# KenHBS/LDA_thesis

Measured on AMD Instinct MI355X. Metric: million tokens resampled/sec (Gibbs sweep), higher is better.
Workload: dtype f64-exact (fp32 tier 0 + fp64 tiers: the drawn topic is the fp64 pipeline's)

## Files before the change

### lda_thesis_amd/csrc/kernel_quad.hpp

```cpp
#pragma once

namespace {

constexpr float LLDA_MARGIN0_QUAD = 0x1.ap-18f;
constexpr float QM_L = 1.05f * 32.0f * 0x1p-24f, QM_T = 1.05f * 39.0f * 0x1p-24f, QM_P = 1.05f * 37.0f * 0x1p-24f, QM_TOT = 1.05f * 0.25f * 0x1p-24f;
#define QLDS(arr, rho, t) (arr)[(rho) >> 2][t][(rho) & 3]
constexpr int QT = 32;
#ifdef LLDA_QUAD_PRIO
constexpr int QP_TOP = (LLDA_QUAD_PRIO) / 100 % 10, QP_DEC = (LLDA_QUAD_PRIO) / 10 % 10, QP_BULK = (LLDA_QUAD_PRIO) % 10;
#else
constexpr int QP_TOP = 3, QP_DEC = 0, QP_BULK = 2;
#endif
constexpr int QNT = 128;
#ifdef LLDA_QUAD_PARTS
constexpr int QUAD_PARTS = (LLDA_QUAD_PARTS);
#else
constexpr int QUAD_PARTS = 7;
#endif
constexpr bool QUAD_FULL_LOOP = (QUAD_PARTS & 1) != 0, QUAD_HOOKS_OUT = (QUAD_PARTS & 2) != 0, QUAD_EARLY_DECODE = (QUAD_PARTS & 4) != 0;
template <bool B> struct QuadForm { static constexpr bool value = B; };

template <int LB>
struct QuadGeo {
    static constexpr int LPD = 1 << LB;
    static constexpr int G = 2 * LPD;
    static constexpr int KP = 32 * LPD;
    static constexpr int IS = 3 + LB;
    static constexpr int DPW = 64 / LPD;
    static constexpr uint64_t GM = LPD == 64 ? ~0ull : ((1ull << LPD) - 1);
    static constexpr uint32_t KEY_NONE = 0xFC000u | 31u << 9 | (uint32_t)(KP - 1);
};

template <int LB>
__device__ __forceinline__ int quad_rho(int pos) { return ((pos >> LB) & 0x18) | ((pos & 3) << 1) | ((pos >> 2) & 1); }
constexpr int quad_rho_of(int i, int e, int c) { return 8 * i + 2 * c + e; }

template <int LB>
__device__ __forceinline__ uint32_t quad_min_key(uint32_t key)
{
    if constexpr (LB == 4)
        asm volatile("s_nop 1\n\tv_min_u32_dpp %0, %0, %0 row_ror:8 row_mask:0xf bank_mask:0xf\n\ts_nop 1\n\t"
                     "v_min_u32_dpp %0, %0, %0 row_ror:4 row_mask:0xf bank_mask:0xf\n\ts_nop 1\n\t"
                     "v_min_u32_dpp %0, %0, %0 row_ror:2 row_mask:0xf bank_mask:0xf\n\ts_nop 1\n\t"
                     "v_min_u32_dpp %0, %0, %0 row_ror:1 row_mask:0xf bank_mask:0xf" : "+v"(key));
    else if constexpr (LB == 3)
        asm volatile("s_nop 1\n\tv_min_u32_dpp %0, %0, %0 row_half_mirror row_mask:0xf bank_mask:0xf\n\ts_nop 1\n\t"
                     "v_min_u32_dpp %0, %0, %0 quad_perm:[1,0,3,2] row_mask:0xf bank_mask:0xf\n\ts_nop 1\n\t"
                     "v_min_u32_dpp %0, %0, %0 quad_perm:[2,3,0,1] row_mask:0xf bank_mask:0xf" : "+v"(key));
    else
        asm volatile("s_nop 1\n\tv_min_u32_dpp %0, %0, %0 quad_perm:[1,0,3,2] row_mask:0xf bank_mask:0xf\n\ts_nop 1\n\t"
                     "v_min_u32_dpp %0, %0, %0 quad_perm:[2,3,0,1] row_mask:0xf bank_mask:0xf" : "+v"(key));
    return key;
}

template <int LB>
struct QuadCounts {
    const int (*s_ndk)[QNT][4];
    const int *s_nk0;
    int t;
    int e;
    int g;
    bool st;
    __device__ __forceinline__ int word(int s) const { return QLDS(s_ndk, 8 * (s >> 2) + 2 * (s & 3) + e, t); }
    __device__ __forceinline__ int nd(int s) const { return word(s) & 0xffff; }
    __device__ __forceinline__ int nk(int s) const
    {
        const int w = word(s);
        return s_nk0[pos_of<QuadGeo<LB>::G, 16>(g, s)] + (w & 0xffff) - (int)((uint32_t)w >> 16);
    }
    __device__ __forceinline__ bool stats() const { return st; }
    __device__ __forceinline__ bool count_unsure() const { return false; }
};

template <int LB, bool PAD>
__device__ __noinline__ int quad_cold(const int (*s_ndk)[QNT][4], const int *s_nk0, int tbase, int w, int f, int zo, uint32_t ra,
                                      uint32_t rb, int lane, int64_t d, const KParams *P)
{
    constexpr int G = QuadGeo<LB>::G;
    const int g = lane & (G - 1);
    int x[16];
    gload_lane_row<G, 16>(P->n_kw, (int64_t)w * QuadGeo<LB>::KP, g, x);
    int lo, so;
    lane_slot_of<G, 16>(zo, lo, so);
#pragma unroll
    for (int s = 0; s < 16; ++s) x[s] -= (g == lo && s == so) ? f : 0;
    const QuadCounts<LB> dc{s_ndk, s_nk0, tbase + (g >> 1), g & 1, g, lane < G};
    if constexpr (PAD) return cold_tiers_acc<G, 16, true, false>(dc, x, P->lab_mask[d * G + g], uniform53(ra, rb), g, lane, P);
    else return cold_tiers_acc<G, 16, false, true>(dc, x, 0xFFFFu, uniform53(ra, rb), g, lane, P);
// ... 29 lines not shown
        tot += dpp_f32<DPP_ROW_ROR + 8>(tot);
        tot += dpp_f32<DPP_ROW_ROR + 4>(tot);
        tot += dpp_f32<DPP_ROW_ROR + 2>(tot);
        tot += dpp_f32<DPP_ROW_ROR + 1>(tot);
        prev = __int_as_float(__builtin_amdgcn_update_dpp(0, __float_as_int(X), DPP_ROW_SHR + 1, 0xF, 0xF, true));
    } else {
        const float m1 = lq >= 1 ? 1.0f : 0.0f, m2 = lq >= 2 ? 1.0f : 0.0f;
        X = __builtin_fmaf(dpp_f32<DPP_ROW_SHR + 1>(X), m1, X);
        X = __builtin_fmaf(dpp_f32<DPP_ROW_SHR + 2>(X), m2, X);
        if constexpr (LB == 3) {
            const float m4 = lq >= 4 ? 1.0f : 0.0f;
            X = __builtin_fmaf(dpp_f32<DPP_ROW_SHR + 4>(X), m4, X);
            tot += dpp_f32<DPP_HALF_MIRROR>(tot);
        }
        tot += dpp_f32<DPP_XOR1>(tot);
        tot += dpp_f32<DPP_XOR2>(tot);
        prev = dpp_f32<DPP_ROW_SHR + 1>(X) * m1;
    }
    LLDA_MARK("threshold");
    const float t = u * tot;
    const float tg = t - prev;
    const float md = __builtin_fmaf(QM_L, X0, __builtin_fmaf(QM_T, t, __builtin_fmaf(QM_P, prev, QM_TOT * tot)));
    float margin = md;
    if constexpr (HOOKS) margin = __builtin_fmaf(tot, margin_rel, margin_data * md);
    const float lo0 = tg - margin, hi0 = tg + margin;
    LLDA_MARK("search");
    const bool c0 = Q[15].x <= lo0;
    const float dA = c0 ? Q[15].x : 0.0f;
    const float lo = lo0 - dA, hi = hi0 - dA;
    float q[16];
#pragma unroll
    for (int a = 0; a < 16; ++a) q[a] = c0 ? Q[a].y : Q[a].x;
    const bool c5 = q[15] <= lo;
    float ub = c5 ? __int_as_float(0x7f800000) : q[15];
    const bool c1 = q[7] <= lo;
    ub = c1 ? ub : q[7];
    const float m2 = c1 ? q[11] : q[3];
    const float a1 = c1 ? q[9] : q[1], a5 = c1 ? q[13] : q[5];
    const float e0 = c1 ? q[8] : q[0], e2 = c1 ? q[10] : q[2], e4 = c1 ? q[12] : q[4], e6 = c1 ? q[14] : q[6];
    const bool c2 = m2 <= lo;
    ub = c2 ? ub : m2;
    const float m3 = c2 ? a5 : a1;
    const float g0 = c2 ? e4 : e0, g2 = c2 ? e6 : e2;
    const bool c3 = m3 <= lo;
    ub = c3 ? ub : m3;
    const float m4 = c3 ? g2 : g0;
    const bool c4 = m4 <= lo;
    ub = c4 ? ub : m4;
    uint64_t bad_total;
    asm("v_cmp_class_f32_e64 %0, %1, %2" : "=s"(bad_total) : "v"(tot - margin), "v"(0x2FF));
    uint64_t unsure = __ballot(!(ub > hi)) | bad_total;
    LLDA_MARK("pick");
    constexpr uint32_t I1 = 2u << QuadGeo<LB>::IS, I0 = 1u << QuadGeo<LB>::IS;
    const uint32_t p = (c1 ? (I1 | 16u << 9) : 0u) | (c2 ? (I0 | 8u << 9) : 0u) | (c3 ? (2u | 4u << 9) : 0u) | (c4 ? (1u | 2u << 9) : 0u) |
                       (c0 ? (4u | 1u << 9) : 0u) | ((uint32_t)lq << 3) | ((uint32_t)lq << 14);
    uint32_t key = c5 ? QuadGeo<LB>::KEY_NONE : p;
    key = quad_min_key<LB>(key);
    zn = (int)(key & 0x3FFFu);
    if constexpr (PAD) unsure |= __ballot(key == QuadGeo<LB>::KEY_NONE);
    return unsure;
}

template <int LB, bool PAD = false>
__device__ __forceinline__ uint64_t quad_tier1(const q_v32f &xv, const int (*s_ndk)[QNT][4], const int *s_nk0, int tid, int lq, double u,
                                               double alpha, double beta, double vbeta, double margin_rel, uint32_t vm, int &zn)
{
    double W[QT];
    double run = 0.0;
#pragma unroll
    for (int k = 0; k < QT; ++k) {
        const int e = k >> 4, a = k & 15, i = a >> 2, c = a & 3;
        const int rho = quad_rho_of(i, e, c);
        const int w = QLDS(s_ndk, rho, tid);
        const int nd = w & 0xffff, nk = s_nk0[(i << QuadGeo<LB>::IS) | (lq << 3) | (e << 2) | c] + nd - (int)((uint32_t)w >> 16);
        const double den = (double)nk + vbeta;
        double y = (double)__builtin_amdgcn_rcpf((float)den);
        y = __builtin_fma(__builtin_fma(-den, y, 1.0), y, y);
        y = __builtin_fma(__builtin_fma(-den, y, 1.0), y, y);
        const double ws = ((double)nd + alpha) * (((double)xv[rho] + beta) * y);
        run = run + (((vm >> k) & 1u) ? ws : 0.0);
        W[k] = run;
    }
    constexpr int LPD = QuadGeo<LB>::LPD;
    const double X = group_scan<LPD>(run, lq);
    const double tot = bcast_last<LPD>(X, tid & 63);
    double prev = dpp_f64<DPP_ROW_SHR + 1>(X);
    if constexpr (LB < 4) prev = lq ? prev : 0.0;
    const double tg = u * tot - prev;
    const double margin = tot * margin_rel;
    const double lo = tg - margin, hi = tg + margin;
    int cnt_lo = 0, cnt_hi = 0;
#pragma unroll
    for (int k = 0; k < QT; ++k) {
        cnt_lo += (W[k] <= lo) ? 1 : 0;
        cnt_hi += (W[k] <= hi) ? 1 : 0;
    }
    uint64_t unsure = __ballot((cnt_lo != cnt_hi) || !(tot > 0.0) || !(margin < tot));
    const uint32_t k = (uint32_t)cnt_lo;
    const uint32_t i_ = (k >> 2) & 3u, e_ = (k >> 4) & 1u, c_ = k & 3u;
    const uint32_t p = (i_ << QuadGeo<LB>::IS) | ((uint32_t)lq << 3) | (e_ << 2) | c_ | ((8u * i_ + 2u * c_ + e_) << 9) | ((uint32_t)lq << 14);
    uint32_t key = cnt_lo >= QT ? QuadGeo<LB>::KEY_NONE : p;
    key = quad_min_key<LB>(key);
    zn = (int)(key & 0x3FFFu);
    if constexpr (PAD) unsure |= __ballot(key == QuadGeo<LB>::KEY_NONE);
    return unsure;
}

struct QuadSite { int v, f, zo, c, zn, lo, so; uint8_t w; };

#ifdef QUAD_PROFILE
#define QP_DECL uint32_t qp_t = 0, qp_acc[8] = {0, 0, 0, 0, 0, 0, 0, 0}
#define QP_START() do { __builtin_amdgcn_sched_barrier(0); qp_t = (uint32_t)__builtin_amdgcn_s_memtime(); __builtin_amdgcn_sched_barrier(0); } while (0)
#define QP_MARK(k) do { __builtin_amdgcn_sched_barrier(0); const uint32_t qp_n = (uint32_t)__builtin_amdgcn_s_memtime(); \
                        qp_acc[k] += qp_n - qp_t; qp_t = qp_n; __builtin_amdgcn_sched_barrier(0); } while (0)
#else
#define QP_DECL
#define QP_START()
#define QP_MARK(k)
#endif

template <int LB, bool REC = (LB < 4), bool PAD = false, bool HOOKS = false>
__global__ void __launch_bounds__(QNT, 2) llda_sweep_quad_kernel(const KParams P)
{
    typedef QuadGeo<LB> Geo;
    constexpr int KP = Geo::KP, LPD = Geo::LPD, G = Geo::G, IS = Geo::IS;
    __shared__ int s_nk[KP];
    __shared__ int s_nk0[KP];
    __shared__ int s_ndk[QT / 4][QNT][4];
    __shared__ float s_pa[QT / 4][QNT][4];
    __shared__ float s_u[QNT / LPD][2 * LPD];
    __shared__ __attribute__((aligned(16))) int s_hot[QT][16];
    static_assert(LB != 4 || sizeof(s_nk) + sizeof(s_nk0) + sizeof(s_ndk) + sizeof(s_pa) + sizeof(s_u) + sizeof(s_hot) <= 40960,
                  "K = 512: the static LDS of a workgroup must leave room for four workgroups on a CU");

    const int tid = threadIdx.x;
    for (int i = tid; i < KP; i += QNT) {
        s_nk[i] = 0;
        s_nk0[i] = P.n_k[i];
    }
    for (int i = tid; i < QT * 16; i += QNT) {
        const int so = i >> 4, k = i & 15;
        const int kk = ((so & 1) << 3) | ((so >> 4) << 2) | (((so >> 3) & 1) << 1) | ((so >> 2) & 1);
        s_hot[so][k] = k == kk ? -(1 << (((so >> 1) & 1) << 4)) : 0;
    }
    __syncthreads();

    const int lane = tid & 63, lq = tid & (LPD - 1), row = lane >> LB, grp = tid >> LB;
    const int gbase = lane & (64 - LPD);
    const float vbeta32 = (float)P.vbeta, alpha32 = (float)P.alpha, beta32 = (float)P.beta;

    const int64_t site_base = P.doc_off[0];
    const int32_t *word_b = P.word + site_base, *freq_b = P.freq + site_base, *csc_b = P.csc_pos + site_base;
    int32_t *z_b = P.z + site_base;

    typedef int v4i __attribute__((ext_vector_type(4)));
    QP_DECL;

    auto update = [&](int sg, int pos, int df) {
        const int w = QLDS(s_ndk, sg, tid) + df;
        QLDS(s_ndk, sg, tid) = w;
        const int nd = w & 0xffff, nk = s_nk0[pos] + nd - (int)((uint32_t)w >> 16);
        QLDS(s_pa, sg, tid) = tier0_factor(nd, nk, alpha32, vbeta32);
    };

    for (int it = 0; it < P.dpg; ++it) {
        const int64_t idx = ((int64_t)blockIdx.x * P.dpg + it) * (QNT / LPD) + grp;
        const bool valid = idx < P.D;
        const int64_t ic = valid ? idx : P.D - 1;
        const int64_t d = P.doc_order ? (int64_t)P.doc_order[ic] : ic;
        int64_t s0 = P.doc_off[d];
        int len = valid ? (int)(P.doc_off[d + 1] - s0) : 0;
        if (len <= 0) {
            len = 0;
            s0 = site_base;
        }
        int maxlen, minlen;
        if constexpr (LB == 4) {
            const int l0 = __builtin_amdgcn_readlane(len, 0), l1 = __builtin_amdgcn_readlane(len, 16);
            const int l2 = __builtin_amdgcn_readlane(len, 32), l3 = __builtin_amdgcn_readlane(len, 48);
            maxlen = max(max(l0, l1), max(l2, l3));
            minlen = min(min(l0, l1), min(l2, l3));
        } else {
            int ml = len, nl = len;
#pragma unroll
            for (int m = LPD; m < 64; m <<= 1) {
                ml = max(ml, __shfl_xor(ml, m, 64));
                nl = min(nl, __shfl_xor(nl, m, 64));
            }
            maxlen = __builtin_amdgcn_readfirstlane(ml);
            minlen = __builtin_amdgcn_readfirstlane(nl);
        }
        if (maxlen == 0) continue;

        int32_t *ndk_row = P.n_dk + d * KP;
        const uint32_t vm = PAD ? (uint32_t)P.lab_mask[d * G + 2 * lq] | (uint32_t)P.lab_mask[d * G + 2 * lq + 1] << 16 : ~0u;
        {
            int big = 0, tokens = 0;
#pragma unroll
            for (int i = 0; i < 4; ++i) {
                const v4i a = ((const v4i *)ndk_row)[i * G + 2 * lq], b = ((const v4i *)ndk_row)[i * G + 2 * lq + 1];
                const int r[8] = {a.x, a.y, a.z, a.w, b.x, b.y, b.z, b.w};
#pragma unroll
                for (int j = 0; j < 8; ++j) {
                    const int rho = quad_rho_of(i, j >> 2, j & 3);
                    const int k = s_nk0[(i << IS) + lq * 8 + j];
                    QLDS(s_ndk, rho, tid) = r[j] | (r[j] << 16);
                    QLDS(s_pa, rho, tid) = ((vm >> (16 * (j >> 2) + 4 * i + (j & 3))) & 1u) ? tier0_factor(r[j], k, alpha32, vbeta32) : 0.0f;
                    big |= r[j];
                    tokens += (int)((uint32_t)r[j] & 0xffffu);
                }
            }
#pragma unroll
            for (int m = 1; m < LPD; m <<= 1) tokens += __shfl_xor(tokens, m, LPD);
            if (valid && (((uint32_t)big >> 16) || tokens > 65535) && P.status) atomicOr(P.status, 4);
        }
        const uint32_t gdoc = (uint32_t)(d + P.doc_base);
        const uint32_t sb = (uint32_t)(s0 - site_base) * 4u;
        const int last = len > 0 ? len - 1 : 0;
        auto off_of = [&](int n) { return opaque_u32(sb + (uint32_t)min(n, last) * 4u); };
        auto off_full = [&](int n) { return opaque_u32(sb + (uint32_t)n * 4u); };
        auto load_scalars = [&](QuadSite &R, const uint32_t o) {
            R.v = gload_i32(word_b, o); R.f = gload_i32(freq_b, o); R.c = gload_i32(csc_b, o); R.zo = gload_i32(z_b, o);
        };
        const int32_t *rec_b = REC ? P.site_rec + site_base * 4 : nullptr;
        int pv = 0, pf = 0, pc = 0;
        auto load_rec = [&](int &v, int &f, int &c, const uint32_t o) {
            const v4i r = *(const LLDA_GLOBAL v4i *)((const LLDA_GLOBAL char *)rec_b + (o << 2));
            v = r.x; f = r.y; c = r.z;
        };
        auto decode_old = [&](QuadSite &R) {
            R.lo = (R.zo >> 3) & (LPD - 1);
            R.so = quad_rho<LB>(R.zo);
        };
        int xp[16];
        auto load_row16 = [&](const int v, uint8_t &flag) {
#ifdef ABL_NOLOAD
#pragma unroll
            for (int k = 0; k < 16; ++k) xp[k] = ((v + k) & 7) * 0x10001;
            flag = 1;
            return;
#endif
            const LLDA_GLOBAL char *q = (const LLDA_GLOBAL char *)P.n_kw16 + (((uint32_t)v << (IS + 3)) + (uint32_t)lq * 16u);
            const v4i a = *(const LLDA_GLOBAL v4i *)q, b = *(const LLDA_GLOBAL v4i *)(q + 32 * LPD);
            const v4i c = *(const LLDA_GLOBAL v4i *)(q + 16 * LPD), e = *(const LLDA_GLOBAL v4i *)(q + 48 * LPD);
            xp[0] = a.x; xp[1] = a.y; xp[2] = a.z; xp[3] = a.w;
            xp[4] = b.x; xp[5] = b.y; xp[6] = b.z; xp[7] = b.w;
            xp[8] = c.x; xp[9] = c.y; xp[10] = c.z; xp[11] = c.w;
            xp[12] = e.x; xp[13] = e.y; xp[14] = e.z; xp[15] = e.w;
            flag = *(const LLDA_GLOBAL uint8_t *)((const LLDA_GLOBAL char *)P.row16 + (uint32_t)v);
        };
        q_v32f xv;
        auto convert_row = [&](const int v, const uint8_t flag, const int so, const float own) {
            LLDA_MARK("convert");
            const uint64_t wide_w = __ballot(flag == 0);
            if (__builtin_expect(wide_w == 0, 1)) {
#pragma unroll
                for (int k = 0; k < 16; ++k) {
                    const int e = k >> 3, j = (k >> 2) & 1, m = k & 3;
                    const int i = 2 * j + (m >> 1), c = 2 * (m & 1);
                    xv[quad_rho_of(i, e, c)] = (float)((uint32_t)xp[k] & 0xffffu);
                    xv[quad_rho_of(i, e, c + 1)] = (float)((uint32_t)xp[k] >> 16);
                }
            } else {
                LLDA_MARK("rare_wide_row");
                int xi[QT];
#pragma unroll
                for (int t = 0; t < QT; ++t) xi[t] = 0;
                if (flag == 0) {
                    const LLDA_GLOBAL v4i *q = (const LLDA_GLOBAL v4i *)((const LLDA_GLOBAL int32_t *)P.n_kw + ((uint64_t)(uint32_t)v << (IS + 2)));
#pragma unroll
                    for (int i = 0; i < 4; ++i) {
                        const v4i a = q[i * G + 2 * lq], b = q[i * G + 2 * lq + 1];
                        xi[quad_rho_of(i, 0, 0)] = a.x; xi[quad_rho_of(i, 0, 1)] = a.y; xi[quad_rho_of(i, 0, 2)] = a.z; xi[quad_rho_of(i, 0, 3)] = a.w;
                        xi[quad_rho_of(i, 1, 0)] = b.x; xi[quad_rho_of(i, 1, 1)] = b.y; xi[quad_rho_of(i, 1, 2)] = b.z; xi[quad_rho_of(i, 1, 3)] = b.w;
                    }
                }
#pragma unroll
                for (int k = 0; k < 16; ++k) {
                    const int e = k >> 3, j = (k >> 2) & 1, m = k & 3;
                    const int i = 2 * j + (m >> 1), c = 2 * (m & 1);
                    const int ra_ = quad_rho_of(i, e, c), rb_ = quad_rho_of(i, e, c + 1);
                    xv[ra_] = flag == 0 ? (float)xi[ra_] : (float)((uint32_t)xp[k] & 0xffffu);
                    xv[rb_] = flag == 0 ? (float)xi[rb_] : (float)((uint32_t)xp[k] >> 16);
                }
#pragma unroll
                for (int r = 0; r < QT; ++r) xv[r] -= (flag == 0 && so == r) ? own : 0.0f;
            }
        };
        auto remove_own_packed = [&](const int so, const int own) {
            LLDA_MARK("own_removal");
            const v4i *hot = (const v4i *)&s_hot[so][0];
#pragma unroll
            for (int j = 0; j < 4; ++j) {
                const v4i h = hot[j];
                xp[4 * j] += __mul24(h.x, own); xp[4 * j + 1] += __mul24(h.y, own);
                xp[4 * j + 2] += __mul24(h.z, own); xp[4 * j + 3] += __mul24(h.w, own);
            }
        };

        QuadSite R0, R1, R2;
        int wq = 0;
        if constexpr (REC) {
            load_rec(R0.v, R0.f, R0.c, off_of(0)); R0.zo = gload_i32(z_b, off_of(0));
            load_rec(R1.v, R1.f, R1.c, off_of(1)); R1.zo = gload_i32(z_b, off_of(1));
            load_rec(pv, pf, pc, off_of(2));
        } else {
            load_scalars(R0, off_of(0));
            load_scalars(R1, off_of(1));
            wq = gload_i32(word_b, off_of(2));
        }
        R0.zn = R1.zn = 0;
        R2.v = R2.f = R2.zo = R2.c = R2.zn = R2.lo = R2.so = R2.w = 0;
        if constexpr (QUAD_EARLY_DECODE) {
            R2.v = REC ? pv : wq;
            R2.zo = gload_i32(z_b, off_of(2));
        }
        load_row16(R0.v, R0.w);
        uint32_t r0 = 0, r1 = 0, r2 = 0, r3 = 0;
        decode_old(R0);
        if constexpr (QUAD_EARLY_DECODE) decode_old(R1);
        if (len > 0 && lq == R0.lo) update(R0.so, R0.zo, -R0.f);
        remove_own_packed(R0.so, (len > 0 && lq == R0.lo) ? R0.f : 0);
        convert_row(R0.v, R0.w, R0.so, (len > 0 && lq == R0.lo) ? (float)R0.f : 0.0f);
        load_row16(R1.v, R1.w);

        auto site = [&](auto form, const int n, QuadSite &cur, QuadSite &nxt, QuadSite &prv) {
            constexpr bool FULL = decltype(form)::value;
            const bool act = FULL || n < len, more = FULL || n + 1 < len;
            auto off = [&](int m) { if constexpr (FULL) return off_full(m); else return off_of(m); };
            const int f = cur.f, zo = cur.zo;
            QP_START();
            if constexpr (FULL || !QUAD_FULL_LOOP) {
                LLDA_MARK("site_top");
            } else {
                LLDA_MARK("site_top_masked");
            }
            LLDA_MARK("lds_factors");
            __builtin_amdgcn_s_setprio(QP_TOP);
            q_v2f pa[16];
#pragma unroll
            for (int a = 0; a < 16; ++a) {
                pa[a].x = QLDS(s_pa, 2 * a, tid);
                pa[a].y = QLDS(s_pa, 2 * a + 1, tid);
            }
            LLDA_MARK("rng");
            if ((n & (2 * LPD - 1)) == 0) {
                LLDA_MARK("rare_philox");
                r0 = (uint32_t)(n >> 1) + (uint32_t)lq; r1 = gdoc; r2 = P.stream_id; r3 = P.sweep;
                philox4x32_10(r0, r1, r2, r3, P.key0, P.key1);
                s_u[grp][2 * lq] = (float)(r0 >> 5) * 0x1p-27f;
                s_u[grp][2 * lq + 1] = (float)(r2 >> 5) * 0x1p-27f;
                LLDA_MARK("rng");
            }
            const float u32 = s_u[grp][n & (2 * LPD - 1)];
            QP_MARK(0);
            int zn;
            uint64_t unsure;
            if constexpr (HOOKS) unsure = quad_draw<LB, PAD, true>(xv, pa, u32, P.margin0_rel, P.margin0_data, beta32, lq, zn);
            else unsure = quad_draw<LB, PAD, false>(xv, pa, u32, 0.0f, 1.0f, beta32, lq, zn);
            if constexpr (!FULL) unsure &= __ballot(act);
            QP_MARK(1);
            LLDA_MARK("cold_check");
            if (__builtin_expect(unsure != 0, 0)) {
                LLDA_MARK("rare_cold");
                const int holder = (n >> 1) & (LPD - 1);
                const uint32_t ra_l = (n & 1) ? r2 : r0, rb_l = (n & 1) ? r3 : r1;
                const int bp_h = (gbase | holder) << 2;
                const uint32_t ra = (uint32_t)__builtin_amdgcn_ds_bpermute(bp_h, (int)ra_l), rb = (uint32_t)__builtin_amdgcn_ds_bpermute(bp_h, (int)rb_l);
                const uint64_t t0_w = unsure;
                if (lq == 0 && ((t0_w >> gbase) & Geo::GM) && P.status) atomicAdd(P.status + 1, 1);
                int z1;
                uint64_t still = ((!HOOKS || P.margin_rel < 1.0 ? quad_tier1<LB, PAD>(xv, s_ndk, s_nk0, tid, lq, uniform53(ra, rb), P.alpha, P.beta, P.vbeta,
                                                                                  P.margin_rel, vm, z1) : ~0ull) | __ballot(cur.w == 0));
                if constexpr (!FULL) still &= __ballot(act);
                const bool mine0 = ((t0_w >> gbase) & Geo::GM) != 0;
                zn = mine0 ? z1 : zn;
                uint32_t rows = 0;
#pragma unroll
                for (int r = 0; r < Geo::DPW; ++r)
                    rows |= (((t0_w >> (LPD * r)) & Geo::GM) && ((still >> (LPD * r)) & Geo::GM)) ? (1u << r) : 0u;
                rows = (uint32_t)__builtin_amdgcn_readfirstlane((int)rows);
                while (__builtin_expect(rows != 0, 0)) {
                    const int r = __builtin_ctz(rows);
                    rows &= rows - 1;
                    const int src = r * LPD;
                    const int zo_r = __builtin_amdgcn_readlane(zo, src);
                    int zc = quad_cold<LB, PAD>(s_ndk, s_nk0, (tid & 64) + src, __builtin_amdgcn_readlane(cur.v, src),
                                       __builtin_amdgcn_readlane(f, src), zo_r, (uint32_t)__builtin_amdgcn_readlane((int)ra, src),
                                       (uint32_t)__builtin_amdgcn_readlane((int)rb, src), lane,
                                       (int64_t)__builtin_amdgcn_readlane((int)d, src),
                                       (const KParams *)__builtin_amdgcn_kernarg_segment_ptr());
                    if (__builtin_expect(zc < 0, 0)) {
                        zc = zo_r;
                        if (lane == 0 && P.status) atomicOr(P.status, 1);
                    }
                    zn = (row == r) ? (zc | (quad_rho<LB>(zc) << 9)) : zn;
                }
            }
            QP_MARK(2);
            LLDA_MARK("decode");

            {
                const int zpos = zn & 511, sn = zn >> 9, ln = (zn >> 3) & (LPD - 1);
                cur.zn = zpos;
                uint32_t cword = (uint32_t)zo | ((uint32_t)zpos << 16);
                asm volatile("" : "+v"(cword));
                if constexpr (!QUAD_EARLY_DECODE) decode_old(nxt);
                const bool own_new = act && lq == ln, own_old = more && lq == nxt.lo;
                const int sg = own_new ? sn : own_old ? nxt.so : 0;
                const int ps = own_new ? zpos : own_old ? nxt.zo : (lq << 3);
                const int df = own_new ? f : own_old ? -nxt.f : 0;
                LLDA_MARK("count_update");
                const int w0 = QLDS(s_ndk, sg, tid), k0 = s_nk0[ps];
                QP_MARK(3);
                LLDA_MARK("scalars");
                __builtin_amdgcn_s_setprio(QP_BULK);
                int w_next;
                if constexpr (REC) {
                    prv.v = w_next = pv; prv.f = pf; prv.c = pc;
                    if constexpr (QUAD_EARLY_DECODE) cur.zo = gload_i32(z_b, off(n + 3));
                    else prv.zo = gload_i32(z_b, off(n + 2));
                    load_rec(pv, pf, pc, off(n + 3));
                } else if constexpr (QUAD_EARLY_DECODE) {
                    w_next = prv.v;
                    prv.f = gload_i32(freq_b, off(n + 2)); prv.c = gload_i32(csc_b, off(n + 2));
                    cur.v = gload_i32(word_b, off(n + 3)); cur.zo = gload_i32(z_b, off(n + 3));
                } else {
                    w_next = wq;
                    load_scalars(prv, off(n + 2));
                    wq = gload_i32(word_b, off(n + 3));
                }
                if constexpr (QUAD_EARLY_DECODE) decode_old(prv);
                QP_MARK(4);
                remove_own_packed(nxt.so, (more && lq == nxt.lo) ? nxt.f : 0);
                convert_row(nxt.v, nxt.w, nxt.so, (more && lq == nxt.lo) ? (float)nxt.f : 0.0f);
                QP_MARK(5);
                LLDA_MARK("row_prefetch");
                load_row16(w_next, prv.w);
                LLDA_MARK("count_update");
                const int w = w0 + df;
                QLDS(s_ndk, sg, tid) = w;
                const int nd = w & 0xffff, nk = k0 + nd - (int)((uint32_t)w >> 16);
                QLDS(s_pa, sg, tid) = tier0_factor(nd, nk, alpha32, vbeta32);
                if (__builtin_expect(__ballot(own_new && own_old) != 0, 0)) {
                    LLDA_MARK("rare_second_update");
                    if (own_new && own_old) update(nxt.so, nxt.zo, -nxt.f);
                }
#ifndef ABL_NOCOMMIT
                {
                    LLDA_MARK("commit");
                    const uint32_t zoff = opaque_u32(sb + (uint32_t)n * 4u);
                    const LLDA_GLOBAL uint32_t *lp = (const LLDA_GLOBAL uint32_t *)P.commit_log + (uint32_t)(cur.c & 0x7fffffff);
                    const uint32_t word = cword;
                    if (lq == 0 && act) {
                        gstore_i32(z_b, zoff, zpos);
                        *(LLDA_GLOBAL uint32_t *)lp = word;
                    }
                }
#endif
            }
            LLDA_MARK("loop");
            QP_MARK(6);
        };
        int n = 0;
        if constexpr (QUAD_FULL_LOOP) {
            for (; n + 5 < minlen; n += 3) {
                site(QuadForm<true>{}, n, R0, R1, R2);
                site(QuadForm<true>{}, n + 1, R1, R2, R0);
                site(QuadForm<true>{}, n + 2, R2, R0, R1);
            }
        }
        for (;; n += 3) {
            site(QuadForm<false>{}, n, R0, R1, R2);
            if (n + 1 >= maxlen) break;
            site(QuadForm<false>{}, n + 1, R1, R2, R0);
            if (n + 2 >= maxlen) break;
            site(QuadForm<false>{}, n + 2, R2, R0, R1);
            if (n + 3 >= maxlen) break;
        }

#ifdef QUAD_PROFILE
        if (blockIdx.x == 0 && tid == 0 && P.status) {
#pragma unroll
            for (int k = 0; k < 8; ++k) atomicAdd(P.status + 8 + k, (int)qp_acc[k]);
            atomicAdd(P.status + 16, maxlen);
        }
#endif
        if (valid && len > 0) {
#pragma unroll
            for (int i = 0; i < 4; ++i) {
                int o[8];
#pragma unroll
                for (int j = 0; j < 8; ++j) {
                    const int w = QLDS(s_ndk, quad_rho_of(i, j >> 2, j & 3), tid);
                    o[j] = w & 0xffff;
                    const int dl = o[j] - (int)((uint32_t)w >> 16);
                    if (dl) atomicAdd(&s_nk[(i << IS) + lq * 8 + j], dl);
                }
                v4i a = {o[0], o[1], o[2], o[3]}, b = {o[4], o[5], o[6], o[7]};
                ((v4i *)ndk_row)[i * G + 2 * lq] = a;
                ((v4i *)ndk_row)[i * G + 2 * lq + 1] = b;
            }
        }
    }

    __syncthreads();
    for (int i = tid; i < KP; i += QNT) {
        const int dl = s_nk[i];
        if (dl) atomicAdd(P.n_k_delta + i, dl);
// ... 28 lines not shown
```

### lda_thesis_amd/csrc/llda_gibbs.hip

```cpp
#include <hip/hip_runtime.h>
#include "build_info.hpp"
#ifndef ABL_EXTRA_LDS_BYTES
#define ABL_EXTRA_LDS_BYTES 0
#endif
#include <stdint.h>
#include <math.h>
#include <string.h>
#include <map>
#include <memory>
#include <type_traits>

#include "llda_gibbs.h"

#pragma clang fp contract(off)

#include "device_common.hpp"
#include "draw_tiers.hpp"
#include "exact_generic.hpp"
#include "kernel_sweep.hpp"
#include "kernel_quad.hpp"
#include "kernel_sparse.hpp"
#include "kernel_batch.hpp"
#include "kernel_readout.hpp"
#include "kernel_foldin.hpp"
// ... 503 lines not shown
            rl = allow_lds(llda_sweep_wide_kernel<true>, lds);
            if (rl) return rl;
            hipLaunchKernelGGL(llda_sweep_wide_kernel<true>, grid, block, lds, st, W);
        } else {
            rl = allow_lds(llda_sweep_wide_kernel<false>, lds);
            if (rl) return rl;
            hipLaunchKernelGGL(llda_sweep_wide_kernel<false>, grid, block, lds, st, W);
        }
#undef LLDA_WIDE_REG
        const hipError_t e = hipGetLastError();
        return e == hipSuccess ? LLDA_OK : hip_fail(e);
    }

    const bool sparse = fast && !dense && a->live_off && a->live_pos && a->live_max >= 1 && a->live_max <= LLDA_MAX_LIVE;
    const int G = sparse ? (a->live_max <= 8 ? 8 : a->live_max <= 16 ? 16 : a->live_max <= 32 ? 32 : 64) : L.G;
    const int gpb = 256 / G;
    int dpg = a->docs_per_group;
    if (dpg < 1) dpg = 1;
    P.dpg = dpg;
    const int64_t per_block = (int64_t)gpb * dpg;
    const int64_t blocks = (a->D + per_block - 1) / per_block;
    if (blocks > 0x7fffffffLL) return LLDA_E_BAD_ARG;

    if (sparse) {
        P.live_off = a->live_off; P.live_pos = a->live_pos;
        if (a->debug_margin < 0) {
            P.margin_rel = 2.0;
            P.margin0_rel = 2.0f;
        }
        const dim3 grid((unsigned)blocks), block(256);
        const int rimg = take_image(a, P);
        if (rimg) return rimg;
#define LLDA_SPARSE(GS_)                                                                                              \
    case GS_:                                                                                                         \
        if (a->img_bits == 8) hipLaunchKernelGGL((llda_sweep_sparse_kernel<GS_, KParams, 8>), grid, block, 0, st, P);       \
        else if (a->img_bits == 16) hipLaunchKernelGGL((llda_sweep_sparse_kernel<GS_, KParams, 16>), grid, block, 0, st, P); \
        else hipLaunchKernelGGL((llda_sweep_sparse_kernel<GS_, KParams, 0>), grid, block, 0, st, P);                       \
        break;
        switch (G) { LLDA_SPARSE(8) LLDA_SPARSE(16) LLDA_SPARSE(32) LLDA_SPARSE(64) }
#undef LLDA_SPARSE
        const hipError_t e = hipGetLastError();
        return e == hipSuccess ? LLDA_OK : hip_fail(e);
    }
    if (a->n_kw_img || a->img_bits) return LLDA_E_BAD_ARG;
    if (a->row16) {
        if (!a->n_kw16 || a->site_row) return LLDA_E_BAD_ARG;
        if (!(fast && a->dense_mask != 0 && logged && llda_quad_ok(a->K))) return LLDA_E_BAD_ARG;
        if (a->D >= (1LL << 31)) return LLDA_E_BAD_ARG;
        P.quad_pad = L.K != L.KP;
        if (P.quad_pad && !P.lab_mask) return LLDA_E_BAD_ARG;
        if (!(a->max_doc_tokens > 0 && a->max_doc_tokens < 65536)) return LLDA_E_BAD_ARG;
        if ((reinterpret_cast<uintptr_t>(a->n_kw16) | reinterpret_cast<uintptr_t>(a->n_kw)) & 15) return LLDA_E_BAD_ARG;
        if (a->V >= (1LL << 22)) return LLDA_E_BAD_ARG;
        if (L.G <= 16 && !P.site_rec) return LLDA_E_BAD_ARG;
        if (a->n_sites < 1) return LLDA_OK;
        P.n_kw16 = a->n_kw16;
        P.row16 = a->row16;
        if (a->debug_margin == 0) {
            P.margin0_rel = 0.0f;
            P.margin0_data = 1.0f;
        } else if (a->debug_margin == -9) {
            P.margin0_rel = LLDA_MARGIN0_QUAD;
            P.margin_rel = 0x1p-40;
        } else if (a->debug_margin <= -10 && a->debug_margin >= -18) {
            P.margin0_rel = 0.0f;
            P.margin0_data = a->debug_margin == -10 ? 1.0f / 1.05f : ldexpf(1.0f, a->debug_margin + 10);
            P.margin_rel = 0x1p-40;
        }
        const int64_t per_q = (int64_t)(2 * QNT / L.G) * dpg;
        const int64_t qblocks = (a->D + per_q - 1) / per_q;
        if (qblocks > 0x7fffffffLL) return LLDA_E_BAD_ARG;
        const dim3 qgrid((unsigned)qblocks), qblock(QNT);
        const bool hooks = a->debug_margin != 0 || !QUAD_HOOKS_OUT;
#define LLDA_QUAD(LB_, REC_, PAD_)                                                                                                    \
        do {                                                                                                                           \
            if (hooks) hipLaunchKernelGGL((llda_sweep_quad_kernel<LB_, REC_, PAD_, true>), qgrid, qblock, 0, st, P);                   \
            else hipLaunchKernelGGL((llda_sweep_quad_kernel<LB_, REC_, PAD_, false>), qgrid, qblock, 0, st, P);                        \
        } while (0)
        if (!P.quad_pad) {
            if (L.G == 32) LLDA_QUAD(4, false, false);
            else if (L.G == 16) LLDA_QUAD(3, true, false);
            else LLDA_QUAD(2, true, false);
        } else {
            if (L.G == 32) LLDA_QUAD(4, false, true);
            else if (L.G == 16) LLDA_QUAD(3, true, true);
            else LLDA_QUAD(2, true, true);
        }
#undef LLDA_QUAD
        const hipError_t e = hipGetLastError();
        return e == hipSuccess ? LLDA_OK : hip_fail(e);
    }
    if ((a->n_kw16 != nullptr) != (a->site_row != nullptr)) return LLDA_E_BAD_ARG;
    if (a->n_kw16) {
        if (!(fast && dense && logged && L.T == 16 && L.G >= 32)) return LLDA_E_BAD_ARG;
        if ((reinterpret_cast<uintptr_t>(a->n_kw16) | reinterpret_cast<uintptr_t>(a->n_kw)) & 15) return LLDA_E_BAD_ARG;
        P.n_kw16 = a->n_kw16;
        P.site_row = a->site_row;
        P.w4 = a->max_doc_tokens > 0 && a->max_doc_tokens < 65536 && a->debug_margin != -8;
    }
    switch (L.G) {
    case 8: return dispatch_sweep_T<8>(L.T, P, has_tail, fast, dense, blocks, st);
    case 16: return dispatch_sweep_T<16>(L.T, P, has_tail, fast, dense, blocks, st);
    case 32: return dispatch_sweep_T<32>(L.T, P, has_tail, fast, dense, blocks, st);
    case 64: return dispatch_sweep_T<64>(L.T, P, has_tail, fast, dense, blocks, st);
    }
    return LLDA_E_BAD_K;
// ... 367 lines not shown
```

### lda_thesis_amd/sampler.py

```python
import os

import numpy as np
import torch

from . import _native
from .layout import group_layout


def shard_documents(doc_off, world_size):
    doc_off = np.asarray(doc_off, dtype=np.int64)
    D = doc_off.shape[0] - 1
    total = int(doc_off[-1])
    bounds = [0]
    for r in range(1, world_size):
        target = total * r // world_size
        b = int(np.searchsorted(doc_off, target, side="left"))
        bounds.append(min(max(b, bounds[-1]), D))
    bounds.append(D)
    return bounds


def _dist_active(group):
    import torch.distributed as dist
    return dist.is_available() and dist.is_initialized() and dist.get_world_size(group) > 1
# ... 218 lines not shown
        def lines_per_site(column):
            n_lines = (KP + per_line - 1) // per_line
            key = torch.unique(docs * n_lines + column // per_line)
            per_doc = torch.bincount(key // n_lines, minlength=self.D).to(torch.float32)
            return float((per_doc * lens).sum().item() / max(float(lens.sum().item()), 1.0))
        self.image_lines_per_site = (lines_per_site(pos), lines_per_site(col_t[pos]))
        if force is not True and self.image_lines_per_site[1] > 0.9 * self.image_lines_per_site[0]:
            return
        self._img_src = torch.from_numpy(src.astype(np.int32)).to(dev)
        self._img_col = col_t.to(torch.int32)

    QUAD_MAX_WIDE_SITES = 0.02
    QUAD_CHECK_EVERY = 32

    def _quad_policy(self):
        if self.sweeps_done % self.QUAD_CHECK_EVERY:
            return
        ev = self._wide_event
        if ev is not None:
            ev.synchronize()
            self._wide_event = None
            if float(self._wide_host[0]) > self.QUAD_MAX_WIDE_SITES * self.S:
                self.quad = False
                self.row16 = None
                if _native.rows16_ok(self.K):
                    self._flag_rows16()
                else:
                    self.n_kw16 = None
                return
        if self._wide_host is None:
            self._wide_host = torch.zeros((1,), dtype=torch.float32).pin_memory()
        share = ((1.0 - self.row16.to(torch.float32)) * self._word_sites).sum().reshape(1)
        self._wide_host.copy_(share, non_blocking=True)
        self._wide_event = torch.cuda.Event()
        self._wide_event.record()

    ROWS16_MIN_BYTES = 64 << 20
    MAX_FREQ = 1 << 23
    PAIR_LIMIT = 32767

    def _make_rows16(self, auto=False):
        V, KP = self.V, self.layout.KP
        if KP % 8:
            raise _native.NativeError("llda_rows16_ok(%d) holds but KP = %d is not a multiple of 8" % (self.K, KP))
        if (V + 1) * (KP // 4) + V * (KP // 8) >= 1 << 31:
            if auto:
                return
            raise ValueError("rows16=True: n_kw of %d x %d is too large for the 32-bit row offsets of the 16-bit-row kernel"
                             % (V, KP))
        tokens_max = int(min(int(self.n_dk.sum(dim=1, dtype=torch.int64).max().item()), 2 ** 31 - 1)) if self.D else 0
        four_waves = 0 < tokens_max < 65536
        if auto and not four_waves and V * KP * 4 < self.ROWS16_MIN_BYTES:
            return
        quad = bool(self._quad_wanted is not False and four_waves and _native.quad_ok(self.K) and V < (1 << 22))
        two_doc = _native.rows16_ok(self.K)
        if quad and self._quad_wanted is None:
            wide = (self.n_kw.max(dim=1).values > 65535) | (self.n_kw.min(dim=1).values < 0)
            self._word_sites = torch.bincount(self.word.to(torch.int64), minlength=V).to(torch.float32)
            if float((wide.to(torch.float32) * self._word_sites).sum().item()) > self.QUAD_MAX_WIDE_SITES * self.S:
                quad = False
        if self._quad_wanted and not quad:
            raise ValueError("quad=True: needs a K with llda_quad_ok (16 slots per lane in 8, 16 or 32 lanes: K = 100, 128, 200, 256, 400, 512 ...), "
                             "documents of fewer than 65 536 tokens and a vocabulary below 2^22 words")
        if not quad and not (two_doc and bool(self._rows16_fits().any())):
            return
        n32 = (V + 1) * KP
        try:
            both = torch.zeros((n32 + V * KP // 2,), dtype=torch.int32, device=self.device)
        except torch.cuda.OutOfMemoryError:
            if not auto:
                raise
            import warnings
            warnings.warn("GibbsSampler: no room for the 16-bit image of n_kw (%.1f GB); sweeping with int32 rows"
                          % (V * KP * 2 / 1e9))
            return
        both[:n32] = self._counts
        self._counts = both[:n32]
        self.n_kw = self._counts[:V * KP].view(V, KP)
        self.n_k = self._counts[V * KP:]
        self._counts16 = both
        self.n_kw16 = both[n32:].view(torch.int16)
        self.quad = quad
        if self.quad:
            self.row16 = torch.zeros((V,), dtype=torch.uint8, device=self.device)
            self.max_doc_tokens = tokens_max
            return
        self._flag_rows16()
        if not self.max_doc_tokens:
            self.max_doc_tokens = tokens_max

    def _rows16_fits(self):
        return (self.n_kw.sum(dim=1, dtype=torch.int64) <= 65535) & (self.n_kw.min(dim=1).values >= 0)

    def _flag_rows16(self):
        KP = self.layout.KP
        fits = self._rows16_fits()
        self.row16 = fits.to(torch.uint8).contiguous()
        w = self.word.to(torch.int64)
        flagged = fits[w]
        self.csc_pos &= 0x7fffffff
        self.csc_pos |= torch.where(flagged, -(1 << 31), 0).to(torch.int32)
        gap = self.n_kw16.data_ptr() - self.n_kw.data_ptr()
        if gap != (self.V + 1) * KP * 4 or gap % 16:
            raise _native.NativeError("n_kw16 is not in the allocation of n_kw")
        self.site_row = torch.where(flagged, gap // 16 + w * (KP // 8), w * (KP // 4)).to(torch.int32).contiguous()

    def _make_exchange_rows(self):
        import torch.distributed as dist
        dev, KP = self.device, self.layout.KP
        mass = torch.zeros((self.V,), dtype=torch.int64, device=dev)
        if self.S:
            mass.index_add_(0, self.word.to(torch.int64), self.freq.to(torch.int64))
        everyone = torch.tensor([1 if (self.commit_log is not None or self.S == 0) else 0], device=dev)
        if _dist_active(self.group):
            dist.all_reduce(mass, group=self.group)
            dist.all_reduce(everyone, op=dist.ReduceOp.MIN, group=self.group)
# ... 412 lines not shown
```

Before: 9128.

## Encode LDS byte offsets in slot keys and use table-driven decode in quad sweep

Replaces the slot index carried in the pick key with a precomputed entry that holds the byte offsets of the count/factor pair and the hot row in LDS, so address arithmetic in the hot update and own-removal paths collapses to a mask and add. Adds an optional LDS lookup table for decoding old topics, and a small-index mode that hoists the collision ballot and uses a 32-bit commit-log offset, with a new site-count limit guarding it. It costs an extra LDS table and a wider key, and restricts quad use to fewer than 2^30 sites.

```diff
diff --git a/lda_thesis_amd/csrc/kernel_quad.hpp b/lda_thesis_amd/csrc/kernel_quad.hpp
--- a/lda_thesis_amd/csrc/kernel_quad.hpp
+++ b/lda_thesis_amd/csrc/kernel_quad.hpp
@@ -15,9 +15,10 @@
 #ifdef LLDA_QUAD_PARTS
 constexpr int QUAD_PARTS = (LLDA_QUAD_PARTS);
 #else
-constexpr int QUAD_PARTS = 7;
+constexpr int QUAD_PARTS = 55;
 #endif
 constexpr bool QUAD_FULL_LOOP = (QUAD_PARTS & 1) != 0, QUAD_HOOKS_OUT = (QUAD_PARTS & 2) != 0, QUAD_EARLY_DECODE = (QUAD_PARTS & 4) != 0;
+constexpr bool QUAD_ENTRY = (QUAD_PARTS & 8) != 0, QUAD_TABLE = (QUAD_PARTS & 16) != 0, QUAD_SMALL = (QUAD_PARTS & 32) != 0;
 template <bool B> struct QuadForm { static constexpr bool value = B; };
 
 template <int LB>
@@ -28,12 +29,35 @@
     static constexpr int IS = 3 + LB;
     static constexpr int DPW = 64 / LPD;
     static constexpr uint64_t GM = LPD == 64 ? ~0ull : ((1ull << LPD) - 1);
-    static constexpr uint32_t KEY_NONE = 0xFC000u | 31u << 9 | (uint32_t)(KP - 1);
 };
 
 template <int LB>
 __device__ __forceinline__ int quad_rho(int pos) { return ((pos >> LB) & 0x18) | ((pos & 3) << 1) | ((pos >> 2) & 1); }
 constexpr int quad_rho_of(int i, int e, int c) { return 8 * i + 2 * c + e; }
+
+constexpr uint32_t QE_NDK = 0x380Cu, QE_HOT = 0x7C0u;
+constexpr uint32_t quad_entry(uint32_t rho) { return ((rho >> 2) * 2048u + (rho & 3u) * 4u) | rho << 6; }
+constexpr uint32_t quad_slot(uint32_t rho) { return QUAD_ENTRY ? quad_entry(rho) : rho; }
+constexpr int QS_BITS = QUAD_ENTRY ? 14 : 5;
+constexpr int QK_LANE = 9 + QS_BITS;
+constexpr uint32_t QK_ZN = (1u << QK_LANE) - 1;
+template <int LB> constexpr uint32_t QUAD_KEY_NONE = 0x3Fu << QK_LANE | quad_slot(31) << 9 | (uint32_t)(QuadGeo<LB>::KP - 1);
+constexpr bool quad_entry_ok()
+{
+    uint32_t seen_or = 0;
+    for (uint32_t r = 0; r < 32; ++r) {
+        const uint32_t en = quad_entry(r);
+        if ((en & ~(QE_NDK | QE_HOT)) || (en & QE_HOT) != r << 6 || (en & QE_NDK) != (r >> 2) * 2048u + (r & 3u) * 4u) return false;
+        for (uint32_t q = 0; q < r; ++q)
+            if (quad_entry(q) == en) return false;
+        if (quad_entry(r | 1u) != (en | quad_entry(1)) || quad_entry(r | 8u) != (en | quad_entry(8))) return false;
+        seen_or |= en;
+    }
+    return seen_or == (QE_NDK | QE_HOT);
+}
+static_assert((QE_NDK & QE_HOT) == 0, "the two fields of an entry do not overlap");
+static_assert(quad_entry_ok(), "quad_entry: injective on 0 .. 31, each field recovers its offset, OR of slots = OR of entries");
+static_assert(quad_entry(31) < (1u << 14) && (0x3Fu << QK_LANE | QK_ZN) <= 0x7FFFFFFFu, "the key fits 31 bits");
 
 template <int LB>
 __device__ __forceinline__ uint32_t quad_min_key(uint32_t key)
@@ -169,12 +193,12 @@
     uint64_t unsure = __ballot(!(ub > hi)) | bad_total;
     LLDA_MARK("pick");
     constexpr uint32_t I1 = 2u << QuadGeo<LB>::IS, I0 = 1u << QuadGeo<LB>::IS;
-    const uint32_t p = (c1 ? (I1 | 16u << 9) : 0u) | (c2 ? (I0 | 8u << 9) : 0u) | (c3 ? (2u | 4u << 9) : 0u) | (c4 ? (1u | 2u << 9) : 0u) |
-                       (c0 ? (4u | 1u << 9) : 0u) | ((uint32_t)lq << 3) | ((uint32_t)lq << 14);
-    uint32_t key = c5 ? QuadGeo<LB>::KEY_NONE : p;
+    const uint32_t p = (c1 ? (I1 | quad_slot(16) << 9) : 0u) | (c2 ? (I0 | quad_slot(8) << 9) : 0u) | (c3 ? (2u | quad_slot(4) << 9) : 0u) |
+                       (c4 ? (1u | quad_slot(2) << 9) : 0u) | (c0 ? (4u | quad_slot(1) << 9) : 0u) | ((uint32_t)lq << 3) | ((uint32_t)lq << QK_LANE);
+    uint32_t key = c5 ? QUAD_KEY_NONE<LB> : p;
     key = quad_min_key<LB>(key);
-    zn = (int)(key & 0x3FFFu);
-    if constexpr (PAD) unsure |= __ballot(key == QuadGeo<LB>::KEY_NONE);
+    zn = (int)(key & QK_ZN);
+    if constexpr (PAD) unsure |= __ballot(key == QUAD_KEY_NONE<LB>);
     return unsure;
 }
 
@@ -215,15 +239,23 @@
     uint64_t unsure = __ballot((cnt_lo != cnt_hi) || !(tot > 0.0) || !(margin < tot));
     const uint32_t k = (uint32_t)cnt_lo;
     const uint32_t i_ = (k >> 2) & 3u, e_ = (k >> 4) & 1u, c_ = k & 3u;
-    const uint32_t p = (i_ << QuadGeo<LB>::IS) | ((uint32_t)lq << 3) | (e_ << 2) | c_ | ((8u * i_ + 2u * c_ + e_) << 9) | ((uint32_t)lq << 14);
-    uint32_t key = cnt_lo >= QT ? QuadGeo<LB>::KEY_NONE : p;
+    const uint32_t p = (i_ << QuadGeo<LB>::IS) | ((uint32_t)lq << 3) | (e_ << 2) | c_ | (quad_slot(8u * i_ + 2u * c_ + e_) << 9) | ((uint32_t)lq << QK_LANE);
+    uint32_t key = cnt_lo >= QT ? QUAD_KEY_NONE<LB> : p;
     key = quad_min_key<LB>(key);
-    zn = (int)(key & 0x3FFFu);
-    if constexpr (PAD) unsure |= __ballot(key == QuadGeo<LB>::KEY_NONE);
+    zn = (int)(key & QK_ZN);
+    if constexpr (PAD) unsure |= __ballot(key == QUAD_KEY_NONE<LB>);
     return unsure;
 }
 
 struct QuadSite { int v, f, zo, c, zn, lo, so; uint8_t w; };
+
+struct QuadDocLds {
+    __attribute__((aligned(16))) int ndk[QT / 4][QNT][4];
+    __attribute__((aligned(16))) float pa[QT / 4][QNT][4];
+};
+static_assert(offsetof(QuadDocLds, pa) == sizeof(int) * QT * QNT && sizeof(int) * QT * QNT < 65536 &&
+              (quad_entry(31) & QE_NDK) == (7 * QNT * 4 + 3) * sizeof(int),
+              "the factor of a slot is an immediate offset away from its count; QE_NDK is the offset of QLDS(arr, rho, 0)");
 
 #ifdef QUAD_PROFILE
 #define QP_DECL uint32_t qp_t = 0, qp_acc[8] = {0, 0, 0, 0, 0, 0, 0, 0}
@@ -243,17 +275,20 @@
     constexpr int KP = Geo::KP, LPD = Geo::LPD, G = Geo::G, IS = Geo::IS;
     __shared__ int s_nk[KP];
     __shared__ int s_nk0[KP];
-    __shared__ int s_ndk[QT / 4][QNT][4];
-    __shared__ float s_pa[QT / 4][QNT][4];
+    __shared__ QuadDocLds s_doc;
+    int (*const s_ndk)[QNT][4] = s_doc.ndk;
+    float (*const s_pa)[QNT][4] = s_doc.pa;
     __shared__ float s_u[QNT / LPD][2 * LPD];
     __shared__ __attribute__((aligned(16))) int s_hot[QT][16];
-    static_assert(LB != 4 || sizeof(s_nk) + sizeof(s_nk0) + sizeof(s_ndk) + sizeof(s_pa) + sizeof(s_u) + sizeof(s_hot) <= 40960,
+    __shared__ uint16_t s_ent[QUAD_TABLE ? KP : 1];
+    static_assert(LB != 4 || sizeof(s_nk) + sizeof(s_nk0) + sizeof(s_doc) + sizeof(s_u) + sizeof(s_hot) + (QUAD_TABLE ? sizeof(s_ent) : 0) <= 40960,
                   "K = 512: the static LDS of a workgroup must leave room for four workgroups on a CU");
 
     const int tid = threadIdx.x;
     for (int i = tid; i < KP; i += QNT) {
         s_nk[i] = 0;
         s_nk0[i] = P.n_k[i];
+        if constexpr (QUAD_TABLE) s_ent[i] = (uint16_t)quad_slot((uint32_t)quad_rho<LB>(i));
     }
     for (int i = tid; i < QT * 16; i += QNT) {
         const int so = i >> 4, k = i & 15;
@@ -273,11 +308,18 @@
     typedef int v4i __attribute__((ext_vector_type(4)));
     QP_DECL;
 
+    char *const doc_lane = (char *)&s_doc.ndk[0][tid][0];
+    auto ndk_of = [&](int sg) -> int * {
+        if constexpr (QUAD_ENTRY) return (int *)(doc_lane + ((uint32_t)sg & QE_NDK));
+        else return &QLDS(s_doc.ndk, sg, tid);
+    };
+    auto pa_of = [&](int *nd) -> float * { return (float *)((char *)nd + offsetof(QuadDocLds, pa)); };
     auto update = [&](int sg, int pos, int df) {
-        const int w = QLDS(s_ndk, sg, tid) + df;
-        QLDS(s_ndk, sg, tid) = w;
+        int *const c = ndk_of(sg);
+        const int w = *c + df;
+        *c = w;
         const int nd = w & 0xffff, nk = s_nk0[pos] + nd - (int)((uint32_t)w >> 16);
-        QLDS(s_pa, sg, tid) = tier0_factor(nd, nk, alpha32, vbeta32);
+        *pa_of(c) = tier0_factor(nd, nk, alpha32, vbeta32);
     };
 
     for (int it = 0; it < P.dpg; ++it) {
@@ -347,7 +389,11 @@
         };
         auto decode_old = [&](QuadSite &R) {
             R.lo = (R.zo >> 3) & (LPD - 1);
-            R.so = quad_rho<LB>(R.zo);
+            if constexpr (QUAD_TABLE) {
+                R.so = s_ent[R.zo];
+                asm("" : "+v"(R.so));
+            }
+            else R.so = (int)quad_slot((uint32_t)quad_rho<LB>(R.zo));
         };
         int xp[16];
         auto load_row16 = [&](const int v, uint8_t &flag) {
@@ -401,12 +447,15 @@
                     xv[rb_] = flag == 0 ? (float)xi[rb_] : (float)((uint32_t)xp[k] >> 16);
                 }
 #pragma unroll
-                for (int r = 0; r < QT; ++r) xv[r] -= (flag == 0 && so == r) ? own : 0.0f;
+                for (int r = 0; r < QT; ++r) xv[r] -= (flag == 0 && so == (int)quad_slot(r)) ? own : 0.0f;
             }
         };
         auto remove_own_packed = [&](const int so, const int own) {
             LLDA_MARK("own_removal");
-            const v4i *hot = (const v4i *)&s_hot[so][0];
+            if constexpr (QUAD_SMALL) __builtin_assume((uint32_t)own < 65536u);
+            const v4i *hot;
+            if constexpr (QUAD_ENTRY) hot = (const v4i *)((const char *)&s_hot[0][0] + ((uint32_t)so & QE_HOT));
+            else hot = (const v4i *)&s_hot[so][0];
 #pragma unroll
             for (int j = 0; j < 4; ++j) {
                 const v4i h = hot[j];
@@ -511,7 +560,7 @@
                         zc = zo_r;
                         if (lane == 0 && P.status) atomicOr(P.status, 1);
                     }
-                    zn = (row == r) ? (zc | (quad_rho<LB>(zc) << 9)) : zn;
+                    zn = (row == r) ? (zc | (int)(quad_slot((uint32_t)quad_rho<LB>(zc)) << 9)) : zn;
                 }
             }
             QP_MARK(2);
@@ -524,11 +573,14 @@
                 asm volatile("" : "+v"(cword));
                 if constexpr (!QUAD_EARLY_DECODE) decode_old(nxt);
                 const bool own_new = act && lq == ln, own_old = more && lq == nxt.lo;
+                uint64_t both_w = 0;
+                if constexpr (QUAD_SMALL) both_w = __builtin_amdgcn_ballot_w64(own_new) & __builtin_amdgcn_ballot_w64(own_old);
                 const int sg = own_new ? sn : own_old ? nxt.so : 0;
                 const int ps = own_new ? zpos : own_old ? nxt.zo : (lq << 3);
                 const int df = own_new ? f : own_old ? -nxt.f : 0;
                 LLDA_MARK("count_update");
-                const int w0 = QLDS(s_ndk, sg, tid), k0 = s_nk0[ps];
+                int *const cg = ndk_of(sg);
+                const int w0 = *cg, k0 = s_nk0[ps];
                 QP_MARK(3);
                 LLDA_MARK("scalars");
                 __builtin_amdgcn_s_setprio(QP_BULK);
@@ -556,10 +608,11 @@
                 load_row16(w_next, prv.w);
                 LLDA_MARK("count_update");
                 const int w = w0 + df;
-                QLDS(s_ndk, sg, tid) = w;
+                *cg = w;
                 const int nd = w & 0xffff, nk = k0 + nd - (int)((uint32_t)w >> 16);
-                QLDS(s_pa, sg, tid) = tier0_factor(nd, nk, alpha32, vbeta32);
-                if (__builtin_expect(__ballot(own_new && own_old) != 0, 0)) {
+                *pa_of(cg) = tier0_factor(nd, nk, alpha32, vbeta32);
+                if constexpr (!QUAD_SMALL) both_w = __ballot(own_new && own_old);
+                if (__builtin_expect(both_w != 0, 0)) {
                     LLDA_MARK("rare_second_update");
                     if (own_new && own_old) update(nxt.so, nxt.zo, -nxt.f);
                 }
@@ -567,11 +620,19 @@
                 {
                     LLDA_MARK("commit");
                     const uint32_t zoff = opaque_u32(sb + (uint32_t)n * 4u);
-                    const LLDA_GLOBAL uint32_t *lp = (const LLDA_GLOBAL uint32_t *)P.commit_log + (uint32_t)(cur.c & 0x7fffffff);
                     const uint32_t word = cword;
-                    if (lq == 0 && act) {
-                        gstore_i32(z_b, zoff, zpos);
-                        *(LLDA_GLOBAL uint32_t *)lp = word;
+                    if constexpr (QUAD_SMALL) {
+                        const uint32_t loff = (uint32_t)cur.c << 2;
+                        if (lq == 0 && act) {
+                            gstore_i32(z_b, zoff, zpos);
+                            gstore_i32((int32_t *)P.commit_log, loff, (int)word);
+                        }
+                    } else {
+                        const LLDA_GLOBAL uint32_t *lp = (const LLDA_GLOBAL uint32_t *)P.commit_log + (uint32_t)(cur.c & 0x7fffffff);
+                        if (lq == 0 && act) {
+                            gstore_i32(z_b, zoff, zpos);
+                            *(LLDA_GLOBAL uint32_t *)lp = word;
+                        }
                     }
                 }
 #endif
diff --git a/lda_thesis_amd/csrc/llda_gibbs.hip b/lda_thesis_amd/csrc/llda_gibbs.hip
--- a/lda_thesis_amd/csrc/llda_gibbs.hip
+++ b/lda_thesis_amd/csrc/llda_gibbs.hip
@@ -579,6 +579,7 @@
         if (!(a->max_doc_tokens > 0 && a->max_doc_tokens < 65536)) return LLDA_E_BAD_ARG;
         if ((reinterpret_cast<uintptr_t>(a->n_kw16) | reinterpret_cast<uintptr_t>(a->n_kw)) & 15) return LLDA_E_BAD_ARG;
         if (a->V >= (1LL << 22)) return LLDA_E_BAD_ARG;
+        if (a->n_sites >= (1LL << 30)) return LLDA_E_BAD_ARG;
         if (L.G <= 16 && !P.site_rec) return LLDA_E_BAD_ARG;
         if (a->n_sites < 1) return LLDA_OK;
         P.n_kw16 = a->n_kw16;
diff --git a/lda_thesis_amd/sampler.py b/lda_thesis_amd/sampler.py
--- a/lda_thesis_amd/sampler.py
+++ b/lda_thesis_amd/sampler.py
@@ -294,7 +294,8 @@
         four_waves = 0 < tokens_max < 65536
         if auto and not four_waves and V * KP * 4 < self.ROWS16_MIN_BYTES:
             return
-        quad = bool(self._quad_wanted is not False and four_waves and _native.quad_ok(self.K) and V < (1 << 22))
+        quad = bool(self._quad_wanted is not False and four_waves and _native.quad_ok(self.K) and V < (1 << 22)
+                    and self.S < (1 << 30))
         two_doc = _native.rows16_ok(self.K)
         if quad and self._quad_wanted is None:
             wide = (self.n_kw.max(dim=1).values > 65535) | (self.n_kw.min(dim=1).values < 0)
@@ -303,7 +304,7 @@
                 quad = False
         if self._quad_wanted and not quad:
             raise ValueError("quad=True: needs a K with llda_quad_ok (16 slots per lane in 8, 16 or 32 lanes: K = 100, 128, 200, 256, 400, 512 ...), "
-                             "documents of fewer than 65 536 tokens and a vocabulary below 2^22 words")
+                             "documents of fewer than 65 536 tokens, a vocabulary below 2^22 words and fewer than 2^30 sites")
         if not quad and not (two_doc and bool(self._rows16_fits().any())):
             return
         n32 = (V + 1) * KP
```

After: 9297, median of 6. 1.02x the previous value.
